# MikeWangWZHL/VidIL

Hardware: AMD Instinct MI355X
Metric: frames/sec whole-node (BLIP caption+filt + CLIP visual-token) 224^2 8f/video (higher is better)
Workload: dtype bf16

## Files before the change

### vidil_amd/csrc/common.h

```cpp
#pragma once
#include <hip/hip_runtime.h>
#include <atomic>
#include <stdint.h>
#include <stdio.h>
#include "../../include/vidil_hip.h"

typedef _Float16 f16;
typedef _Float16 f16x4 __attribute__((ext_vector_type(4)));
typedef _Float16 f16x8 __attribute__((ext_vector_type(8)));
typedef __bf16 bf16;
typedef __bf16 bf16x4 __attribute__((ext_vector_type(4)));
typedef __bf16 bf16x8 __attribute__((ext_vector_type(8)));
typedef float f32x2 __attribute__((ext_vector_type(2)));
typedef float f32x4 __attribute__((ext_vector_type(4)));
typedef float f32x16 __attribute__((ext_vector_type(16)));
typedef uint32_t u32x2 __attribute__((ext_vector_type(2)));
typedef uint32_t u32x4 __attribute__((ext_vector_type(4)));

#define VIDIL_WAVE 64

void vidil_set_error(const char* fmt, ...);
int vidil_cu_count();
int vidil_lds_opt_in(std::atomic<unsigned long long>& mask, const void* kern, int bytes, const char* who);
const char* vidil_dev_env(const char* name);

bool vidil_gemm256_eligible(const vidil_gemm_args& a, bool any_size = false);
int vidil_gemm256_launch(const vidil_gemm_args& a, hipStream_t s);
const char* vidil_gemm256_variant(const vidil_gemm_args& a);
bool vidil_gemm4w128_wanted(const vidil_gemm_args& a);
int vidil_gemm4w128_launch(const vidil_gemm_args& a, hipStream_t s);
bool vidil_gemm_c3_serves(const vidil_gemm_args& a);
int vidil_gemm4w_c3_launch(const vidil_gemm_args& a, hipStream_t s);

#define VIDIL_REQUIRE(cond, ...)                \
  do {                                          \
    if (!(cond)) {                              \
      vidil_set_error(__VA_ARGS__);             \
      return VIDIL_EINVAL;                      \
    }                                           \
  } while (0)

#define VIDIL_CHECK_LAUNCH(what)                                            \
  do {                                                                      \
    hipError_t e__ = hipGetLastError();                                     \
    if (e__ != hipSuccess) {                                                \
      vidil_set_error("%s: launch failed: %s", what, hipGetErrorString(e__)); \
      return VIDIL_ELAUNCH;                                                 \
    }                                                                       \
  } while (0)

__host__ __device__ __forceinline__ int vt_pos(int t) { return t ^ ((((t >> 2) ^ (t >> 3)) & 1) * 12); }

__host__ __device__ __forceinline__ size_t ktile_off(int t, int c) {
  return (size_t)(t >> 5) * 2048 + (size_t)(((c >> 3) * 32 + (t & 31)) * 8 + (c & 7));
}
__host__ __device__ __forceinline__ size_t vtile_off(int t, int d) {
  const int tt = t & 31, g = (tt & 15) >> 2;
  return (size_t)(t >> 5) * 2048 +
         (size_t)(((((tt >> 4) * 2 + (d >> 5)) * 2 + (g & 1)) * 32 + (d & 31)) * 8 + (g >> 1) * 4 + (tt & 3));
}

__device__ __forceinline__ float wave_sum(float v) {
#pragma unroll
  for (int o = 32; o > 0; o >>= 1) v += __shfl_xor(v, o, 64);
  return v;
}
__device__ __forceinline__ float wave_max(float v) {
#pragma unroll
  for (int o = 32; o > 0; o >>= 1) v = fmaxf(v, __shfl_xor(v, o, 64));
  return v;
}
__device__ __forceinline__ f16 to_f16(float v) {
  asm volatile("" : "+v"(v));
  return (f16)v;
}

template <typename T> struct Elt;
template <> struct Elt<f16> {
  typedef f16x4 x4;
  typedef f16x8 x8;
  static constexpr int kDtype = VIDIL_DT_F16;
  static __device__ __forceinline__ f32x16 mfma32(x8 a, x8 b, f32x16 c) { return __builtin_amdgcn_mfma_f32_32x32x16_f16(a, b, c, 0, 0, 0); }
  static __device__ __forceinline__ f16 from_f32(float v) { return to_f16(v); }
};
template <> struct Elt<bf16> {
  typedef bf16x4 x4;
  typedef bf16x8 x8;
  static constexpr int kDtype = VIDIL_DT_BF16;
  static __device__ __forceinline__ f32x16 mfma32(x8 a, x8 b, f32x16 c) { return __builtin_amdgcn_mfma_f32_32x32x16_bf16(a, b, c, 0, 0, 0); }
  static __device__ __forceinline__ bf16 from_f32(float v) {
    asm volatile("" : "+v"(v));
    return (bf16)v;
  }
};
struct fp8 { uint8_t bits; };
typedef int i32x8 __attribute__((ext_vector_type(8)));
typedef int i32x4 __attribute__((ext_vector_type(4)));
template <> struct Elt<fp8> {
  static constexpr int kDtype = VIDIL_DT_FP8;
};
__device__ __forceinline__ uint32_t pack4_fp8(float a, float b, float c, float d) {
  a = fminf(fmaxf(a, -448.f), 448.f);
  b = fminf(fmaxf(b, -448.f), 448.f);
  c = fminf(fmaxf(c, -448.f), 448.f);
  d = fminf(fmaxf(d, -448.f), 448.f);
  int w = __builtin_amdgcn_cvt_pk_fp8_f32(a, b, 0, false);
  w = __builtin_amdgcn_cvt_pk_fp8_f32(c, d, w, true);
  return (uint32_t)w;
}

template <typename T> __device__ __forceinline__ typename Elt<T>::x8 zero8() {
  typename Elt<T>::x8 z;
#pragma unroll
  for (int e = 0; e < 8; ++e) z[e] = (T)0.f;
  return z;
}
#define VIDIL_DISPATCH_DTYPE(dtype, what, ...)                                         \
  do {                                                                                 \
    if ((dtype) == VIDIL_DT_F16) { using T = f16; __VA_ARGS__; }                       \
    else if ((dtype) == VIDIL_DT_BF16) { using T = bf16; __VA_ARGS__; }                \
    else { vidil_set_error("%s: unknown dtype %d", what, (int)(dtype)); return VIDIL_EINVAL; } \
  } while (0)

__device__ __forceinline__ f32x2 pk_fma(f32x2 a, f32x2 b, f32x2 c) { return __builtin_elementwise_fma(a, b, c); }
__device__ __forceinline__ f32x2 pk_splat(float v) { return f32x2{v, v}; }
__device__ __forceinline__ f32x2 gelu_erf2(f32x2 x) {
  const f32x2 xs = x * pk_splat(0.70710678118654752440f);
  const f32x2 ax = __builtin_elementwise_abs(xs);
  const f32x2 den = pk_fma(pk_splat(0.3275911f), ax, pk_splat(1.0f));
  const f32x2 t = {__builtin_amdgcn_rcpf(den[0]), __builtin_amdgcn_rcpf(den[1])};
  f32x2 p = pk_fma(pk_splat(1.061405429f), t, pk_splat(-1.453152027f));
  p = pk_fma(p, t, pk_splat(1.421413741f));
  p = pk_fma(p, t, pk_splat(-0.284496736f));
  p = pk_fma(p, t, pk_splat(0.254829592f));
  const f32x2 arg = (ax * ax) * pk_splat(-1.4426950408889634f);
  const f32x2 e = {__builtin_amdgcn_exp2f(arg[0]), __builtin_amdgcn_exp2f(arg[1])};
  const f32x2 y = pk_fma(-(p * t), e, pk_splat(1.0f));
  const f32x2 er = {copysignf(y[0], xs[0]), copysignf(y[1], xs[1])};
  return (x * pk_splat(0.5f)) * (er + pk_splat(1.0f));
}
template <typename TO> struct GeluPoly;
template <> struct GeluPoly<f16> {
  static constexpr int DEG = 8;
  static constexpr float q[9] = {3.988192516e-01f, -6.619034771e-02f, 9.718823738e-03f, -1.079092217e-03f, 8.849158500e-05f,
                                 -5.147754456e-06f, 1.986294828e-07f, -4.515713104e-09f, 4.547582994e-11f};
};
template <> struct GeluPoly<bf16> {
  static constexpr int DEG = 6;
  static constexpr float q[7] = {3.978833846e-01f, -6.457313509e-02f, 8.772395999e-03f, -8.140167550e-04f, 4.795563103e-05f,
                                 -1.598607122e-06f, 2.278152054e-08f};
};
template <typename TO>
__device__ __forceinline__ float gelu_fast1(float x) {
  using P = GeluPoly<TO>;
  const float s = x * x;
  float p = __builtin_fmaf(P::q[P::DEG], s, P::q[P::DEG - 1]);
#pragma unroll
  for (int k = P::DEG - 2; k >= 0; --k) p = __builtin_fmaf(p, s, P::q[k]);
  const float phi = __builtin_amdgcn_fmed3f(__builtin_fmaf(x, p, 0.5f), 0.f, 1.f);
  return x * phi;
}
template <typename TO>
__device__ __forceinline__ f32x2 gelu_fast2(f32x2 x) { return f32x2{gelu_fast1<TO>(x[0]), gelu_fast1<TO>(x[1])}; }
__device__ __forceinline__ f32x2 pk_fma_half_clamp(f32x2 a, f32x2 b) {
  f32x2 d;
  asm("v_pk_fma_f32 %0, %1, %2, 0.5 op_sel_hi:[1,1,0] clamp" : "=v"(d) : "v"(a), "v"(b));
  return d;
}
template <typename TO, int NP>
__device__ __forceinline__ void gelu_fast2p_n(f32x2 (&x)[NP]) {
  using P = GeluPoly<TO>;
  f32x2 s[NP], p[NP];
#pragma unroll
  for (int i = 0; i < NP; ++i) s[i] = x[i] * x[i];
#pragma unroll
  for (int i = 0; i < NP; ++i) p[i] = pk_fma(pk_splat(P::q[P::DEG]), s[i], pk_splat(P::q[P::DEG - 1]));
#pragma unroll
  for (int k = P::DEG - 2; k >= 0; --k)
#pragma unroll
    for (int i = 0; i < NP; ++i) p[i] = pk_fma(p[i], s[i], pk_splat(P::q[k]));
#pragma unroll
// ... 12 lines not shown
```

### vidil_amd/csrc/gemm256.hip

```cpp
#include <type_traits>

#include "common.h"
#include "gemm_epilogue.h"

namespace {

constexpr int SLOT = 16384;
constexpr int BUF = 4 * SLOT;
constexpr int LDS_BYTES = 2 * BUF;
constexpr int STATS_BYTES = 2 * 4 * 128 * 8;

__device__ __forceinline__ void glds16(const void* g, char* lds) {
  __builtin_amdgcn_global_load_lds((const __attribute__((address_space(1))) void*)g,
                                   (__attribute__((address_space(3))) void*)lds, 16, 0, 0);
}

template <int EPI>
constexpr bool kPersistent = EPI != VIDIL_EPI_HEADS && EPI != VIDIL_EPI_ARENA;

#ifdef VIDIL_GEMM_PROBE
__device__ unsigned long long g_probe[2];
struct Probe {
  unsigned long long t0, r0;
  __device__ Probe() : t0(__builtin_readcyclecounter()), r0(__builtin_amdgcn_s_memrealtime()) {}
// ... 147 lines not shown
        if (ks == 0) { dma_piece(h, 0); dma_piece(h, 1); dma_piece(h, 2); }
      }
    }
  };

  auto prologue = [&]() {
    issue(baseW, gW[0], 0, 2);
    issue(baseW, gW[1], 0, 3);
    issue(baseA, gA[0], 0, 0);
    issue(baseA, gA[1], 0, 1);
  };
  prologue();

  for (;;) {
#pragma unroll
  for (int it = 0; it < 4; ++it)
#pragma unroll
    for (int j = 0; j < 2; ++j)
#pragma unroll
      for (int r = 0; r < 16; ++r) acc[it][j][r] = 0.f;
  if constexpr (ROWSTAT) {
    const int nparts = (FOLD ? K : N) >> 6;
    const f32x2* stats_in = (const f32x2*)p.ln_stats;
    const int part0 = wc + 4 * hi;
#pragma unroll
    for (int it = 0; it < 4; ++it) {
      int row = m0 + grp * 128 + it * 32 + l31;
      row = row < M ? row : M - 1;
      st_raw[it][0] = part0 < nparts ? stats_in[(size_t)row * nparts + part0] : f32x2{0.f, 0.f};
      st_raw[it][1] = part0 + 8 < nparts ? stats_in[(size_t)row * nparts + part0 + 8] : f32x2{0.f, 0.f};
    }
  }

  int h = 0;
  if (grp == 1) {
    sync(h);
    dma_piece(h, 0); dma_piece(h, 1); dma_piece(h, 2);
    ++h;
  }
  for (int u = 0; u < nk; ++u) {
    const char* buf = smem + (u & 1) * BUF;
    sync(h);
    half_period(std::integral_constant<int, 0>{}, buf, h);
    ++h;
    sync(h);
    half_period(std::integral_constant<int, 1>{}, buf, h);
    ++h;
  }
  if (grp == 0) sync(h);
  asm volatile("s_waitcnt vmcnt(0) lgkmcnt(0)" ::: "memory");
  __builtin_amdgcn_s_barrier();

  if constexpr (ROWSTAT) {
    f32x2* stats = (f32x2*)(smem + LDS_BYTES);
#pragma unroll
    for (int it = 0; it < 4; ++it) {
      const float s0 = st_raw[it][0][0] + st_raw[it][1][0], ss0 = st_raw[it][0][1] + st_raw[it][1][1];
      const float s = s0 + __shfl_xor(s0, 32, 64);
      const float ss = ss0 + __shfl_xor(ss0, 32, 64);
      if (hi == 0) stats[(grp * 4 + wc) * 128 + it * 32 + l31] = f32x2{s, ss};
    }
    asm volatile("s_waitcnt lgkmcnt(0)" ::: "memory");
    __builtin_amdgcn_s_barrier();
    const float inv_k = 1.0f / (float)(FOLD ? K : N);
#pragma unroll
    for (int it = 0; it < 4; ++it) {
      float s = 0.f, ss = 0.f;
#pragma unroll
      for (int w = 0; w < 4; ++w) {
        const f32x2 v = stats[(grp * 4 + w) * 128 + it * 32 + l31];
        s += v[0];
        ss += v[1];
      }
      const float mean = s * inv_k;
      float var = ss * inv_k - mean * mean;
      var = var > 0.f ? var : 0.f;
      const float rstd = 1.0f / sqrtf(var + p.ln_eps);
      st_s[it] = rstd;
      st_ss[it] = mean * rstd;
    }
  }

  const int m_w = m0 + grp * 128;
  const int n_w = n0 + wc * 64;
  const bool more = kPersistent<EPI> && ESZ == 2 && !RLN && remaining > tile_step;
  if (more) {
    logical += tile_step;
    remaining -= tile_step;
    setup_tile(logical);
    prologue();
  }
  do {
    char* const ep = smem + BUF + wave * 8192;
#include "gemm_epilogue.inc"
  } while (0);
  if (!more) break;
  asm volatile("s_waitcnt vmcnt(0) lgkmcnt(0)" ::: "memory");
  }
}

template <typename T, int EPI, int ACT, bool FOLD = false, typename TO = T, bool STATS = false, bool RLN = false>
int launch256(const vidil_gemm_args& a, hipStream_t s) {
  static std::atomic<unsigned long long> attr_set{0};
  auto kern = gemm256_kernel<T, TO, EPI, ACT, FOLD, STATS, RLN>;
  constexpr int lds = LDS_BYTES + ((FOLD || RLN) ? STATS_BYTES : 0);
  if (const int rc_ = vidil_lds_opt_in(attr_set, (const void*)kern, lds, "gemm256")) return rc_;
  const int num_cu = vidil_cu_count() & ~7;
  const int ntiles = ((a.M + 255) / 256) * ((a.N + 255) / 256);
  const int tiles = !(kPersistent<EPI> && sizeof(T) == 2 && !RLN) ? ntiles : ntiles >= num_cu ? num_cu : (ntiles >= 8 ? ((ntiles + 7) & ~7) : ntiles);
  hipLaunchKernelGGL(kern, dim3(tiles), dim3(512), lds, s, a);
  VIDIL_CHECK_LAUNCH("gemm256");
  return VIDIL_OK;
}

}

#ifdef VIDIL_GEMM_PROBE
extern "C" int vidil_debug_gemm_probe(unsigned long long* out2) {
  return hipMemcpyFromSymbol(out2, HIP_SYMBOL(g_probe), 16) == hipSuccess ? 0 : -1;
}
#endif

bool vidil_gemm256_eligible(const vidil_gemm_args& a, bool any_size) {
  const long tiles = (long)((a.M + 255) / 256) * ((a.N + 255) / 256);
  if (tiles < 5L * vidil_cu_count() / 8 && !any_size) return false;
  if (a.K < 128) return false;
  if (a.dtype == VIDIL_DT_FP8 && (a.K % 128 != 0 || (a.lda != 0 && a.lda % 16 != 0))) return false;
  const long lda = a.lda > 0 ? a.lda : a.K;
  if (256L * lda >= (1L << 31) || (long)a.N * a.K >= (1L << 31)) return false;
  auto al16 = [](const void* p) { return ((uintptr_t)p & 15) == 0; };
  if (a.bias && !al16(a.bias)) return false;
  if (a.ln_fold && !(a.ln_colsum && al16(a.ln_colsum) && a.N % 4 == 0 && a.ln_stats && ((uintptr_t)a.ln_stats & 7) == 0)) return false;
  if (a.ln_stats_out && !(a.N % 64 == 0 && ((uintptr_t)a.ln_stats_out & 7) == 0)) return false;
  if (a.w_scale && !al16(a.w_scale)) return false;
  switch (a.epi) {
    case VIDIL_EPI_F8:
      return a.dtype == VIDIL_DT_FP8 && a.N % 16 == 0 && a.ldo % 16 == 0 && al16(a.out);
    case VIDIL_EPI_F16:
      return a.N % 8 == 0 && a.ldo % 8 == 0 && al16(a.out);
    case VIDIL_EPI_F32:
      if (a.out16 && !(a.ldo16 % 4 == 0 && ((uintptr_t)a.out16 & 7) == 0)) return false;
      return a.N % 4 == 0 && a.ldo % 4 == 0 && al16(a.out) && (!a.resid || al16(a.resid));
    case VIDIL_EPI_PATCH:
      return a.N % 4 == 0 && a.ldo % 4 == 0 && al16(a.out) && al16(a.pos);
    case VIDIL_EPI_HEADS:
      return (!a.q || al16(a.q)) && (!a.k || al16(a.k)) && ((a.NP != 0 && !a.kv_tiled) || !a.vt || al16(a.vt));
    case VIDIL_EPI_ARENA:
      return (!a.q || al16(a.q)) && (!a.k || al16(a.k)) && (!a.vt || al16(a.vt));
    default:
      return false;
  }
}

template <typename T>
static int launch256_dispatch(const vidil_gemm_args& a, hipStream_t s) {
  if (a.ln_fold) {
    if (a.epi == VIDIL_EPI_HEADS) return launch256<T, VIDIL_EPI_HEADS, VIDIL_ACT_NONE, true>(a, s);
    if (a.epi == VIDIL_EPI_ARENA) return launch256<T, VIDIL_EPI_ARENA, VIDIL_ACT_NONE, true>(a, s);
    if (a.act == VIDIL_ACT_NONE) return launch256<T, VIDIL_EPI_F16, VIDIL_ACT_NONE, true>(a, s);
    if (a.act == VIDIL_ACT_GELU_ERF) return launch256<T, VIDIL_EPI_F16, VIDIL_ACT_GELU_ERF, true>(a, s);
    return launch256<T, VIDIL_EPI_F16, VIDIL_ACT_QUICK_GELU, true>(a, s);
  }
  switch (a.epi) {
    case VIDIL_EPI_F16:
      if (a.act == VIDIL_ACT_NONE) return launch256<T, VIDIL_EPI_F16, VIDIL_ACT_NONE>(a, s);
      if (a.act == VIDIL_ACT_GELU_ERF) return launch256<T, VIDIL_EPI_F16, VIDIL_ACT_GELU_ERF>(a, s);
      return launch256<T, VIDIL_EPI_F16, VIDIL_ACT_QUICK_GELU>(a, s);
    case VIDIL_EPI_F32:
      if (a.rln_gamma) return launch256<T, VIDIL_EPI_F32, VIDIL_ACT_NONE, false, T, true, true>(a, s);
      if (a.ln_stats_out) return launch256<T, VIDIL_EPI_F32, VIDIL_ACT_NONE, false, T, true>(a, s);
      if (a.act == VIDIL_ACT_NONE) return launch256<T, VIDIL_EPI_F32, VIDIL_ACT_NONE>(a, s);
      if (a.act == VIDIL_ACT_GELU_ERF) return launch256<T, VIDIL_EPI_F32, VIDIL_ACT_GELU_ERF>(a, s);
      return launch256<T, VIDIL_EPI_F32, VIDIL_ACT_QUICK_GELU>(a, s);
    case VIDIL_EPI_HEADS:
      return launch256<T, VIDIL_EPI_HEADS, VIDIL_ACT_NONE>(a, s);
    case VIDIL_EPI_ARENA:
      return launch256<T, VIDIL_EPI_ARENA, VIDIL_ACT_NONE>(a, s);
    default:
      return launch256<T, VIDIL_EPI_PATCH, VIDIL_ACT_NONE>(a, s);
  }
}

template <typename TO>
static int launch256_fp8(const vidil_gemm_args& a, hipStream_t s) {
  switch (a.epi) {
    case VIDIL_EPI_F32: return launch256<fp8, VIDIL_EPI_F32, VIDIL_ACT_NONE, false, TO>(a, s);
    case VIDIL_EPI_PATCH: return launch256<fp8, VIDIL_EPI_PATCH, VIDIL_ACT_NONE, false, TO>(a, s);
    case VIDIL_EPI_HEADS: return launch256<fp8, VIDIL_EPI_HEADS, VIDIL_ACT_NONE, false, TO>(a, s);
    case VIDIL_EPI_F8:
      if (a.act == VIDIL_ACT_GELU_ERF) return launch256<fp8, VIDIL_EPI_F8, VIDIL_ACT_GELU_ERF, false, TO>(a, s);
      if (a.act == VIDIL_ACT_QUICK_GELU) return launch256<fp8, VIDIL_EPI_F8, VIDIL_ACT_QUICK_GELU, false, TO>(a, s);
      return launch256<fp8, VIDIL_EPI_F8, VIDIL_ACT_NONE, false, TO>(a, s);
    default:
      vidil_set_error("gemm/fp8: epilogue %d is not built for fp8 operands", a.epi);
      return VIDIL_EUNSUP;
  }
}

int vidil_gemm4w_launch(const vidil_gemm_args& a, hipStream_t s, int tm);

static bool prefer_4w(const vidil_gemm_args& a) {
  if (a.epi == VIDIL_EPI_HEADS && a.T < 8) return false;
  if (const char* e = vidil_dev_env("VIDIL_GEMM4W")) return atoi(e) != 0;
  const long tiles = (long)((a.M + 255) / 256) * ((a.N + 255) / 256);
  static const long min_tiles = 3L * vidil_cu_count() / 2;
  if (a.dtype == VIDIL_DT_FP8) {
    return tiles >= min_tiles &&
           (a.epi == VIDIL_EPI_F8 || a.epi == VIDIL_EPI_HEADS || (a.epi == VIDIL_EPI_F32 && a.act == VIDIL_ACT_NONE));
  }
  if (tiles < min_tiles) return false;
  if (a.ln_fold) return true;
  switch (a.epi) {
    case VIDIL_EPI_F16:
    case VIDIL_EPI_HEADS:
    case VIDIL_EPI_ARENA:
      return true;
    case VIDIL_EPI_F32: {
      return a.ln_stats_out != nullptr || a.K >= 1536;
    }
    default:
      return false;
  }
}

const char* vidil_gemm256_variant(const vidil_gemm_args& a) { return prefer_4w(a) ? "gemm4w_kernel" : "gemm256_kernel"; }

bool vidil_gemm4w128_wanted(const vidil_gemm_args& a) {
  const char* e = vidil_dev_env("VIDIL_GEMM4W128");
  const int mode = e ? atoi(e) : -1;
  if (mode == 0 || a.dtype == VIDIL_DT_FP8 || a.ln_fold || a.ln_stats_out || a.rln_gamma || a.out16) return false;
  if (a.epi == VIDIL_EPI_HEADS && a.T < 8) return false;
  if (!(a.epi == VIDIL_EPI_F16 || a.epi == VIDIL_EPI_HEADS || a.epi == VIDIL_EPI_ARENA || (a.epi == VIDIL_EPI_F32 && a.act == VIDIL_ACT_NONE)))
    return false;
  if (!vidil_gemm256_eligible(a, true)) return false;
  if (mode == 1) return true;
  const long t256 = (long)((a.M + 255) / 256) * ((a.N + 255) / 256);
  const long t128 = (long)((a.M + 127) / 128) * ((a.N + 255) / 256);
  return t256 < 5L * vidil_cu_count() / 8 && t128 >= 25L * vidil_cu_count() / 32 && a.K >= 512;
}
int vidil_gemm4w128_launch(const vidil_gemm_args& a, hipStream_t s) { return vidil_gemm4w_launch(a, s, 2); }

int vidil_gemm256_launch(const vidil_gemm_args& a, hipStream_t s) {
  if (prefer_4w(a)) {
    const int rc = vidil_gemm4w_launch(a, s, 4);
    if (rc != -1000) return rc;
  }
  if (a.dtype == VIDIL_DT_FP8) return a.dtype16 == VIDIL_DT_BF16 ? launch256_fp8<bf16>(a, s) : launch256_fp8<f16>(a, s);
  if (a.dtype == VIDIL_DT_BF16) return launch256_dispatch<bf16>(a, s);
  return launch256_dispatch<f16>(a, s);
}
```

### vidil_amd/csrc/gemm_epilogue.inc

```
  if (n_w >= N) break;

#ifdef VIDIL_EPI_NIT
  constexpr int NIT = VIDIL_EPI_NIT;
#else
  constexpr int NIT = 4;
#endif
#ifdef VIDIL_EPI_LAZY
  f32x4 q_b[2][4], q_c[2][4];
  const bool has_bias = p.bias != nullptr;
#pragma unroll
  for (int j = 0; j < 2; ++j)
#pragma unroll
    for (int rq = 0; rq < 4; ++rq) {
      q_b[j][rq] = f32x4{0.f, 0.f, 0.f, 0.f};
      q_c[j][rq] = f32x4{0.f, 0.f, 0.f, 0.f};
    }
#ifdef VIDIL_EPI_BIAS_LDS
  constexpr bool VEC_LDS = EPI == VIDIL_EPI_F16 || EPI == VIDIL_EPI_HEADS || EPI == VIDIL_EPI_ARENA || EPI == VIDIL_EPI_F8;
#else
  constexpr bool VEC_LDS = false;
#endif
  if constexpr (VEC_LDS) {
#ifdef VIDIL_EPI_BIAS_LDS
    if (has_bias) {
#pragma unroll
      for (int j = 0; j < 2; ++j)
#pragma unroll
        for (int rq = 0; rq < 4; ++rq) q_b[j][rq] = *(const f32x4*)(epb + (j * 32 + rq * 8 + hi * 4) * 4);
    }
    if constexpr (FOLD || ESZ == 1) {
#pragma unroll
      for (int j = 0; j < 2; ++j)
#pragma unroll
        for (int rq = 0; rq < 4; ++rq) q_c[j][rq] = *(const f32x4*)(epb + 512 + (j * 32 + rq * 8 + hi * 4) * 4);
    }
#endif
  } else {
    if (has_bias) {
#pragma unroll
      for (int j = 0; j < 2; ++j)
#pragma unroll
        for (int rq = 0; rq < 4; ++rq) {
          const int col = n_w + j * 32 + rq * 8 + hi * 4;
          q_b[j][rq] = *(const f32x4*)(p.bias + (col + 4 <= N ? col : N - 4));
        }
    }
    if constexpr (FOLD || ESZ == 1) {
      const float* const cvec = FOLD ? p.ln_colsum : p.w_scale;
#pragma unroll
      for (int j = 0; j < 2; ++j)
#pragma unroll
        for (int rq = 0; rq < 4; ++rq) {
          const int col = n_w + j * 32 + rq * 8 + hi * 4;
          q_c[j][rq] = *(const f32x4*)(cvec + (col + 4 <= N ? col : N - 4));
        }
    }
  }
  auto quadrow = [&](int it, int j, f32x4 (&q4)[4]) {
    f32x2 w[8];
#pragma unroll
    for (int pi = 0; pi < 8; ++pi) {
      const int rq = pi >> 1, e = (pi & 1) * 2;
      w[pi] = f32x2{acc[it][j][rq * 4 + e], acc[it][j][rq * 4 + e + 1]};
      const f32x2 b2 = {q_b[j][rq][e], q_b[j][rq][e + 1]};
      if constexpr (FOLD) {
        const f32x2 c2 = {q_c[j][rq][e], q_c[j][rq][e + 1]};
        w[pi] = pk_fma(w[pi], pk_splat(st_s[it]), pk_fma(pk_splat(-st_ss[it]), c2, b2));
      } else if constexpr (ESZ == 1) {
        const f32x2 c2 = {q_c[j][rq][e], q_c[j][rq][e + 1]};
        w[pi] = pk_fma(w[pi], c2, b2);
      } else {
        w[pi] = w[pi] + b2;
      }
    }
    if constexpr (ACT == VIDIL_ACT_GELU_ERF && EPI != VIDIL_EPI_F32) {
      gelu_fast2p_n<TO, 8>(w);
    } else if constexpr (ACT != VIDIL_ACT_NONE) {
#pragma unroll
      for (int pi = 0; pi < 8; ++pi) w[pi] = ACT == VIDIL_ACT_GELU_ERF ? gelu_erf2(w[pi]) : quick_gelu2(w[pi]);
    }
#pragma unroll
    for (int rq = 0; rq < 4; ++rq) q4[rq] = f32x4{w[rq * 2][0], w[rq * 2][1], w[rq * 2 + 1][0], w[rq * 2 + 1][1]};
  };
#else
  if constexpr (FOLD) {
#pragma unroll
    for (int j = 0; j < 2; ++j)
#pragma unroll
      for (int rq = 0; rq < 4; ++rq) {
        const int col = n_w + j * 32 + rq * 8 + hi * 4;
        if (col + 4 <= N) {
          const f32x4 c4 = *(const f32x4*)(p.ln_colsum + col);
          f32x4 b4 = {0.f, 0.f, 0.f, 0.f};
          if (p.bias != nullptr) b4 = *(const f32x4*)(p.bias + col);
#pragma unroll
          for (int it = 0; it < 4; ++it)
#pragma unroll
            for (int e = 0; e < 4; ++e)
              acc[it][j][rq * 4 + e] = __builtin_fmaf(acc[it][j][rq * 4 + e], st_s[it], __builtin_fmaf(-st_ss[it], c4[e], b4[e]));
        }
      }
  } else if constexpr (ESZ == 1) {
#pragma unroll
    for (int j = 0; j < 2; ++j)
#pragma unroll
      for (int rq = 0; rq < 4; ++rq) {
        const int col = n_w + j * 32 + rq * 8 + hi * 4;
        if (col + 4 <= N) {
          const f32x4 w4 = *(const f32x4*)(p.w_scale + col);
          f32x4 b4 = {0.f, 0.f, 0.f, 0.f};
          if (p.bias != nullptr) b4 = *(const f32x4*)(p.bias + col);
#pragma unroll
          for (int it = 0; it < 4; ++it)
#pragma unroll
            for (int e = 0; e < 4; ++e) acc[it][j][rq * 4 + e] = __builtin_fmaf(acc[it][j][rq * 4 + e], w4[e], b4[e]);
        }
      }
  } else
  if (p.bias != nullptr) {
#pragma unroll
    for (int j = 0; j < 2; ++j)
#pragma unroll
      for (int rq = 0; rq < 4; ++rq) {
        const int col = n_w + j * 32 + rq * 8 + hi * 4;
        if (col + 4 <= N) {
          const f32x4 b4 = *(const f32x4*)(p.bias + col);
#pragma unroll
          for (int it = 0; it < 4; ++it)
#pragma unroll
            for (int e = 0; e < 4; ++e) acc[it][j][rq * 4 + e] += b4[e];
        }
      }
  }
  if constexpr (ACT != VIDIL_ACT_NONE) {
#pragma unroll
    for (int it = 0; it < 4; ++it)
#pragma unroll
      for (int j = 0; j < 2; ++j)
#pragma unroll
        for (int r = 0; r < 16; r += 2) {
          f32x2 v = {acc[it][j][r], acc[it][j][r + 1]};
          v = ACT == VIDIL_ACT_GELU_ERF ? (EPI == VIDIL_EPI_F32 ? gelu_erf2(v) : gelu_fast2<TO>(v)) : quick_gelu2(v);
          acc[it][j][r] = v[0];
          acc[it][j][r + 1] = v[1];
        }
  }
  auto quadrow = [&](int it, int j, f32x4 (&q4)[4]) {
#pragma unroll
    for (int rq = 0; rq < 4; ++rq) q4[rq] = f32x4{acc[it][j][rq * 4 + 0], acc[it][j][rq * 4 + 1], acc[it][j][rq * 4 + 2], acc[it][j][rq * 4 + 3]};
  };
#endif

  int part = 0, head = 0;
  if constexpr (EPI == VIDIL_EPI_HEADS || EPI == VIDIL_EPI_ARENA) {
    const int hd = p.H * 64;
    part = p.part0 + n_w / hd;
    head = (n_w % hd) >> 6;
  }

  if constexpr (EPI == VIDIL_EPI_HEADS) {
    if (part == 2 && p.kv_tiled) {
      constexpr int ROWB = 136;
      const size_t img_stride = (size_t)p.H * p.Tk_cap * 64;
      f16* const vbase = (f16*)p.vt + (size_t)head * p.Tk_cap * 64;
#pragma unroll
      for (int it = 0; it < NIT; ++it) {
        const int mb = m_w + it * 32;
        const int rows = M - mb < 32 ? M - mb : 32;
        if (rows <= 0) break;
#pragma unroll
        for (int j = 0; j < 2; ++j) {
          f32x4 q4[4];
          quadrow(it, j, q4);
#pragma unroll
          for (int rq = 0; rq < 4; ++rq) {
            const f32x4 q = q4[rq];
            const f16x4 v = {Elt<TO>::from_f32(q[0]), Elt<TO>::from_f32(q[1]), Elt<TO>::from_f32(q[2]), Elt<TO>::from_f32(q[3])};
            *(f16x4*)(ep + l31 * ROWB + (j * 32 + rq * 8 + hi * 4) * 2) = v;
          }
        }
        int b = mb / p.T, t = mb - b * p.T;
        for (int r = 0; r < rows;) {
          const int tt = p.t_off + t;
          f16* dst = vbase + (size_t)b * img_stride + vtile_off(tt, lane);
          const char* src = ep + r * ROWB + lane * 2;
          if ((tt & 3) == 0 && r + 4 <= rows && t + 4 <= p.T) {
            const f16x4 v = {*(const f16*)src, *(const f16*)(src + ROWB), *(const f16*)(src + 2 * ROWB),
                             *(const f16*)(src + 3 * ROWB)};
            *(f16x4*)dst = v;
            r += 4;
            t += 4;
          } else {
            *dst = *(const f16*)src;
            r += 1;
            t += 1;
          }
          if (t >= p.T) { t -= p.T; ++b; }
        }
      }
      break;
    }
    if (part == 2 && p.NP != 0) {
#pragma unroll
      for (int it = 0; it < NIT; ++it) {
        const int m = m_w + it * 32 + l31;
        if (m < M) {
          const int b = m / p.T, t = m - b * p.T;
          f16* dst = (f16*)p.vt + (((size_t)b * p.H + head) * 64) * (size_t)p.NP + vt_pos(p.t_off + t);
#pragma unroll
          for (int j = 0; j < 2; ++j) {
            f32x4 q4[4];
            quadrow(it, j, q4);
#pragma unroll
            for (int rq = 0; rq < 4; ++rq) {
              const f32x4 q = q4[rq];
#pragma unroll
              for (int e = 0; e < 4; ++e) dst[(size_t)(j * 32 + rq * 8 + hi * 4 + e) * p.NP] = Elt<TO>::from_f32(q[e]);
            }
          }
        }
      }
      break;
    }
  }

  if constexpr (EPI == VIDIL_EPI_F8) {
#pragma unroll
    for (int pass = 0; pass < 2; ++pass) {
#pragma unroll
      for (int i = 0; i < 2; ++i) {
        const int it = pass * 2 + i;
        const int row = i * 32 + l31;
#pragma unroll
        for (int j = 0; j < 2; ++j) {
          f32x4 q4[4];
          quadrow(it, j, q4);
#pragma unroll
          for (int rq = 0; rq < 4; ++rq) {
            const int cb = j * 32 + rq * 8 + hi * 4;
            const f32x4 q = q4[rq];
            *(uint32_t*)(ep + row * 64 + ((((cb >> 4) ^ ((row >> 2) & 3)) << 4) | (cb & 15))) = pack4_fp8(q[0], q[1], q[2], q[3]);
          }
        }
      }
      const int ch = lane & 3;
#ifdef VIDIL_EPI_LAZY
      const uint32_t pitch8 = (uint32_t)p.ldo;
      const int rows_w8 = M - m_w < 32 * NIT ? M - m_w : 32 * NIT;
      const __amdgpu_buffer_rsrc_t r_o8 = uniform_rsrc((char*)p.out + (size_t)m_w * p.ldo + n_w, (rows_w8 > 0 ? (uint32_t)rows_w8 : 0u) * pitch8);
      uint32_t vo8 = n_w + ch * 16 + 16 <= N ? (uint32_t)(pass * 64 + (lane >> 2)) * pitch8 + (uint32_t)ch * 16u : 0x80000000u;
#pragma unroll
      for (int iter = 0; iter < 4; ++iter) {
        const int row = iter * 16 + (lane >> 2);
        const u32x4 v = *(const u32x4*)(ep + row * 64 + ((ch ^ ((row >> 2) & 3)) << 4));
        __builtin_amdgcn_raw_buffer_store_b128(v, r_o8, vo8, 0, 0);
        vo8 += 16u * pitch8;
      }
#else
#pragma unroll
      for (int iter = 0; iter < 4; ++iter) {
        const int row = iter * 16 + (lane >> 2);
        const i32x4 v = *(const i32x4*)(ep + row * 64 + ((ch ^ ((row >> 2) & 3)) << 4));
        const int m = m_w + pass * 64 + row;
        const int col = n_w + ch * 16;
        if (m < M && col + 16 <= N) *(i32x4*)((char*)p.out + (size_t)m * p.ldo + col) = v;
      }
#endif
    }
  } else if constexpr (EPI == VIDIL_EPI_F16 || EPI == VIDIL_EPI_HEADS || EPI == VIDIL_EPI_ARENA) {
    const float scale = ((EPI == VIDIL_EPI_HEADS || EPI == VIDIL_EPI_ARENA) && part == 0) ? p.q_scale : 1.0f;
#ifdef VIDIL_EPI_LAZY
    {
      const int ch = lane & 7;
      auto compute_write = [&](int it, char* buf) {
#pragma unroll
        for (int j = 0; j < 2; ++j) {
          f32x4 q4[4];
          quadrow(it, j, q4);
#pragma unroll
          for (int rq = 0; rq < 4; ++rq) {
            const f32x4 q = q4[rq];
            const f32x2 q01 = f32x2{q[0], q[1]} * pk_splat(scale), q23 = f32x2{q[2], q[3]} * pk_splat(scale);
            const f16x4 v = {Elt<TO>::from_f32(q01[0]), Elt<TO>::from_f32(q01[1]), Elt<TO>::from_f32(q23[0]), Elt<TO>::from_f32(q23[1])};
            *(f16x4*)(buf + l31 * 128 + (((j * 4 + rq) ^ (l31 & 7)) << 4) + hi * 8) = v;
          }
        }
      };
      auto read_rows = [&](const char* buf, f16x8 (&v4)[4]) {
#pragma unroll
        for (int i = 0; i < 4; ++i) {
          const int row = i * 8 + (lane >> 3);
          v4[i] = *(const f16x8*)(buf + row * 128 + ((ch ^ (row & 7)) << 4));
        }
      };
      f16* hb = nullptr;
      int cap = 0, toff = 0;
      bool tiled = false;
      size_t img = 0;
      if constexpr (EPI == VIDIL_EPI_HEADS) {
        if (part == 0) { hb = (f16*)p.q; cap = p.Tq_cap; toff = 0; tiled = false; }
        else { hb = (f16*)(part == 1 ? p.k : p.vt); cap = p.Tk_cap; toff = p.t_off; tiled = p.kv_tiled != 0; }
        hb += (size_t)head * cap * 64;
        img = (size_t)p.H * cap * 64;
      }
      if constexpr (EPI == VIDIL_EPI_ARENA) {
        hb = (f16*)(part == 0 ? p.q : part == 1 ? p.k : p.vt) + head * 64;
      }
      const bool colok = n_w + ch * 8 + 8 <= N;
      __amdgpu_buffer_rsrc_t r_o16;
      uint32_t vo_o16 = 0, step_o16 = 0;
      if constexpr (EPI == VIDIL_EPI_F16) {
        const uint32_t pitch = (uint32_t)p.ldo * (uint32_t)sizeof(f16);
        const int rows_w = M - m_w < 32 * NIT ? M - m_w : 32 * NIT;
        r_o16 = uniform_rsrc((char*)p.out + ((size_t)m_w * p.ldo + n_w) * sizeof(f16), (rows_w > 0 ? (uint32_t)rows_w : 0u) * pitch);
        vo_o16 = colok ? (uint32_t)(lane >> 3) * pitch + (uint32_t)ch * 16u : 0x80000000u;
        step_o16 = 8u * pitch;
      }
      __amdgpu_buffer_rsrc_t r_hd;
      int hs_b = 0, hs_t = 0, hs_b0 = 0;
      uint32_t img_b = 0;
      if constexpr (EPI == VIDIL_EPI_HEADS) {
        const int b0 = m_w / p.T;
        hs_b0 = b0;
        r_hd = uniform_rsrc((char*)(hb + (size_t)b0 * img), 0x80000000u);
        const int m0l = m_w + (lane >> 3);
        const int bb = m0l / p.T;
        hs_t = m0l - bb * p.T;
        hs_b = bb - b0;
        img_b = (uint32_t)(img * sizeof(f16));
      }
      auto store_rows = [&](int it, f16x8 (&v4)[4]) {
        const int m_first = m_w + it * 32 + (lane >> 3);
        if constexpr (EPI == VIDIL_EPI_F16) {
#pragma unroll
          for (int i = 0; i < 4; ++i) {
            __builtin_amdgcn_raw_buffer_store_b128(__builtin_bit_cast(u32x4, v4[i]), r_o16, vo_o16, 0, 0);
            vo_o16 += step_o16;
          }
        } else if constexpr (EPI == VIDIL_EPI_HEADS) {
          auto rows4 = [&](auto tiled_tag) {
            constexpr bool TILED = decltype(tiled_tag)::value;
#pragma unroll
            for (int i = 0; i < 4; ++i) {
              const int m = m_first + i * 8;
              const uint32_t e = TILED ? (uint32_t)ktile_off(toff + hs_t, ch * 8) : (uint32_t)(toff + hs_t) * 64u + (uint32_t)ch * 8u;
              uint32_t off = (uint32_t)hs_b * img_b + e * (uint32_t)sizeof(f16);
              off = (m < M && colok) ? off : 0x80000000u;
              __builtin_amdgcn_raw_buffer_store_b128(__builtin_bit_cast(u32x4, v4[i]), r_hd, off, 0, 0);
              hs_t += 8;
              const bool wrap = hs_t >= p.T;
              hs_t = wrap ? hs_t - p.T : hs_t;
              hs_b = wrap ? hs_b + 1 : hs_b;
            }
          };
          if (tiled) {
            rows4(std::true_type{});
          } else {
            rows4(std::false_type{});
          }
        } else {
          int b = m_first / p.T, t = m_first - b * p.T;
          const size_t hd = (size_t)p.H * 64;
#pragma unroll
          for (int i = 0; i < 4; ++i) {
            const int m = m_first + i * 8;
            if (m < M && colok) {
              f16* d = hb + (part == 0 ? (size_t)m : (size_t)(p.t_off + t) * p.arena_rows + (size_t)b * p.slot_stride) * hd + ch * 8;
              *(f16x8*)d = v4[i];
            }
            t += 8;
            while (t >= p.T) { t -= p.T; ++b; }
          }
        }
      };
      f16x8 vr[4];
      compute_write(0, ep);
#pragma unroll
      for (int it = 1; it < NIT; ++it) {
        read_rows(ep, vr);
        __builtin_amdgcn_sched_barrier(0);
        compute_write(it, ep);
        __builtin_amdgcn_sched_barrier(0);
        store_rows(it - 1, vr);
        __builtin_amdgcn_sched_barrier(0);
      }
      read_rows(ep, vr);
      store_rows(NIT - 1, vr);
    }
#else
#pragma unroll
    for (int pass = 0; pass < 2; ++pass) {
#pragma unroll
      for (int i = 0; i < 2; ++i) {
        const int it = pass * 2 + i;
        const int row = i * 32 + l31;
#pragma unroll
        for (int j = 0; j < 2; ++j) {
          f32x4 q4[4];
          quadrow(it, j, q4);
#pragma unroll
          for (int rq = 0; rq < 4; ++rq) {
            const f32x4 q = q4[rq];
            const f16x4 v = {Elt<TO>::from_f32(q[0] * scale), Elt<TO>::from_f32(q[1] * scale), Elt<TO>::from_f32(q[2] * scale),
                             Elt<TO>::from_f32(q[3] * scale)};
            *(f16x4*)(ep + row * 128 + (((j * 4 + rq) ^ (row & 7)) << 4) + hi * 8) = v;
          }
        }
      }
      const int ch = lane & 7;
#pragma unroll 4
      for (int iter = 0; iter < 8; ++iter) {
        const int row = iter * 8 + (lane >> 3);
        const f16x8 v = *(const f16x8*)(ep + row * 128 + ((ch ^ (row & 7)) << 4));
        const int m = m_w + pass * 64 + row;
        const int col = n_w + ch * 8;
        if (m < M && col + 8 <= N) {
          if constexpr (EPI == VIDIL_EPI_F16) {
            *(f16x8*)((f16*)p.out + (size_t)m * p.ldo + col) = v;
          } else if constexpr (EPI == VIDIL_EPI_ARENA) {
            const int b = m / p.T, t = m - b * p.T;
            const size_t hd = (size_t)p.H * 64;
            f16* base = (f16*)(part == 0 ? p.q : part == 1 ? p.k : p.vt) + head * 64 + ch * 8;
            *(f16x8*)(base + (part == 0 ? (size_t)m : (size_t)(p.t_off + t) * p.arena_rows + (size_t)b * p.slot_stride) * hd) = v;
          } else {
            const int b = m / p.T, t = m - b * p.T;
            const size_t bh = (size_t)b * p.H + head;
            if (part == 0) {
              *(f16x8*)((f16*)p.q + (bh * p.Tq_cap + t) * 64 + ch * 8) = v;
            } else {
              f16* kv = (f16*)(part == 1 ? p.k : p.vt);
              if (p.kv_tiled) {
                *(f16x8*)(kv + bh * p.Tk_cap * 64 + ktile_off(p.t_off + t, ch * 8)) = v;
              } else {
                *(f16x8*)(kv + (bh * p.Tk_cap + p.t_off + t) * 64 + ch * 8) = v;
              }
            }
          }
        }
      }
    }
#endif
  } else {
    f32x4 rln_g = {1.f, 1.f, 1.f, 1.f}, rln_b = {0.f, 0.f, 0.f, 0.f};
    if constexpr (RLN) {
      const int col = n_w + (lane & 15) * 4;
      if (col + 4 <= N) {
        rln_g = *(const f32x4*)(p.rln_gamma + col);
        rln_b = *(const f32x4*)(p.rln_beta + col);
      }
    }
    if constexpr (EPI == VIDIL_EPI_F32) {
#ifndef VIDIL_EPI_F32_AHEAD
#define VIDIL_EPI_F32_AHEAD 1
#endif
      constexpr int AH = VIDIL_EPI_F32_AHEAD;
      const int ch = lane & 15;
      const uint32_t pitch = (uint32_t)p.ldo * 4u;
      const int rows_w = M - m_w < 32 * NIT ? M - m_w : 32 * NIT;
      const uint32_t nrows = rows_w > 0 ? (uint32_t)rows_w : 0u;
      const size_t e0 = (size_t)m_w * p.ldo + n_w;
      const bool has_res = p.resid != nullptr, has16 = p.out16 != nullptr;
      const bool s3 = !STATS && !RLN && p.out16_split3 != 0;
      const bool s3_third = p.out16_split3 != 2;
      const uint32_t pl16 = (uint32_t)(p.ldo16 / 3) * 2u;
      const __amdgpu_buffer_rsrc_t r_out = uniform_rsrc((char*)p.out + e0 * 4, p.out != nullptr ? nrows * pitch : 0u);
      const __amdgpu_buffer_rsrc_t r_res = uniform_rsrc((const char*)(has_res ? p.resid : (const float*)p.out) + e0 * 4, has_res ? nrows * pitch : 0u);
      const uint32_t pitch16 = (uint32_t)p.ldo16 * 2u;
      const __amdgpu_buffer_rsrc_t r_16 = uniform_rsrc((char*)p.out16 + (has16 ? ((size_t)m_w * p.ldo16 + n_w) * 2 : 0), has16 ? nrows * pitch16 : 0u);
      const bool colok = n_w + ch * 4 + 4 <= N;
      const uint32_t vo0 = colok ? (uint32_t)(lane >> 4) * pitch + (uint32_t)ch * 16u : 0x80000000u;
      const uint32_t vo16_0 = colok ? (uint32_t)(lane >> 4) * pitch16 + (uint32_t)ch * 8u : 0x80000000u;
      f32x4 addb[AH + 1][8];
      uint32_t vo_ld = vo0, vo_st = vo0, vo16 = vo16_0;
      const uint32_t step = 4u * pitch, step16 = 4u * pitch16;
      auto load_rows = [&](f32x4 (&a8)[8]) {
#pragma unroll
        for (int iter = 0; iter < 8; ++iter) {
          a8[iter] = __builtin_bit_cast(f32x4, __builtin_amdgcn_raw_buffer_load_b128(r_res, vo_ld, 0, 0));
          vo_ld += step;
        }
      };
#pragma unroll
      for (int a = 0; a < AH; ++a)
        if (a < NIT) load_rows(addb[a]);
#pragma unroll
      for (int pass = 0; pass < NIT; ++pass) {
        if (pass + AH < NIT) load_rows(addb[(pass + AH) % (AH + 1)]);
        {
          const int it = pass;
          const int lr = l31;
#pragma unroll
          for (int j = 0; j < 2; ++j) {
            f32x4 q4[4];
            quadrow(it, j, q4);
#pragma unroll
            for (int rq = 0; rq < 4; ++rq) *(f32x4*)(ep + lr * 256 + (((j * 8 + rq * 2 + hi) ^ (lr & 7)) << 4)) = q4[rq];
          }
        }
        f32x4 vrow[8];
#pragma unroll
        for (int iter = 0; iter < 8; ++iter) {
          const int lr = iter * 4 + (lane >> 4);
          vrow[iter] = *(const f32x4*)(ep + lr * 256 + ((ch ^ (lr & 7)) << 4));
        }
        float rs8[8], mrs8[8];
        if constexpr (RLN) {
#pragma unroll
          for (int iter = 0; iter < 8; ++iter) {
            const int lr = iter * 4 + (lane >> 4);
            rs8[iter] = __shfl(st_s[pass], lr, 64);
            mrs8[iter] = __shfl(st_ss[pass], lr, 64);
          }
        }
        float part[16];
#pragma unroll
        for (int iter = 0; iter < 8; ++iter) {
          f32x4 v = vrow[iter];
          {
            f32x4 ad = addb[pass % (AH + 1)][iter];
            if constexpr (RLN) {
              const float rs = rs8[iter], mrs = mrs8[iter];
#pragma unroll
              for (int e = 0; e < 4; ++e) ad[e] = __builtin_fmaf(__builtin_fmaf(ad[e], rs, -mrs), rln_g[e], rln_b[e]);
            }
// ... 211 lines not shown
```

Measured before the change: 5136.

## Use buffer stores with running offsets in HEADS/ARENA epilogues for small T

Rewrites the GEMM epilogue row stores for the HEADS and ARENA paths to use buffer-resource stores with precomputed running byte offsets, stepping rows with a batch/time stride so sequence lengths below 8 work. This lets the 4-wave GEMM paths serve HEADS with T<8 (previously excluded), gated by a new check that the arena offset span fits in 31 bits. It also adds an optional lazy V-tile scatter path behind a compile flag. The goal is less per-row index division and branching in the store loop, and more shapes on the faster kernel. The cost is more complex offset arithmetic that could be wrong on edge cases.

```diff
diff --git a/vidil_amd/csrc/common.h b/vidil_amd/csrc/common.h
--- a/vidil_amd/csrc/common.h
+++ b/vidil_amd/csrc/common.h
@@ -27,6 +27,7 @@
 bool vidil_gemm256_eligible(const vidil_gemm_args& a, bool any_size = false);
 int vidil_gemm256_launch(const vidil_gemm_args& a, hipStream_t s);
 const char* vidil_gemm256_variant(const vidil_gemm_args& a);
+bool vidil_gemm4w_arena_fits(const vidil_gemm_args& a);
 bool vidil_gemm4w128_wanted(const vidil_gemm_args& a);
 int vidil_gemm4w128_launch(const vidil_gemm_args& a, hipStream_t s);
 bool vidil_gemm_c3_serves(const vidil_gemm_args& a);
diff --git a/vidil_amd/csrc/gemm256.hip b/vidil_amd/csrc/gemm256.hip
--- a/vidil_amd/csrc/gemm256.hip
+++ b/vidil_amd/csrc/gemm256.hip
@@ -323,6 +323,13 @@
   }
 }
 
+bool vidil_gemm4w_arena_fits(const vidil_gemm_args& a) {
+  if (a.epi != VIDIL_EPI_ARENA || a.T <= 0 || a.H <= 0) return true;
+  if (a.part0 == 0 && a.N <= a.H * 64) return true;
+  const long long span = ((long long)(a.T - 1) * a.arena_rows + (long long)(256 / a.T + 2) * a.slot_stride) * a.H * 128LL;
+  return span < (1LL << 31);
+}
+
 template <typename T>
 static int launch256_dispatch(const vidil_gemm_args& a, hipStream_t s) {
   if (a.ln_fold) {
@@ -371,7 +378,7 @@
 int vidil_gemm4w_launch(const vidil_gemm_args& a, hipStream_t s, int tm);
 
 static bool prefer_4w(const vidil_gemm_args& a) {
-  if (a.epi == VIDIL_EPI_HEADS && a.T < 8) return false;
+  if (!vidil_gemm4w_arena_fits(a)) return false;
   if (const char* e = vidil_dev_env("VIDIL_GEMM4W")) return atoi(e) != 0;
   const long tiles = (long)((a.M + 255) / 256) * ((a.N + 255) / 256);
   static const long min_tiles = 3L * vidil_cu_count() / 2;
@@ -400,7 +407,7 @@
   const char* e = vidil_dev_env("VIDIL_GEMM4W128");
   const int mode = e ? atoi(e) : -1;
   if (mode == 0 || a.dtype == VIDIL_DT_FP8 || a.ln_fold || a.ln_stats_out || a.rln_gamma || a.out16) return false;
-  if (a.epi == VIDIL_EPI_HEADS && a.T < 8) return false;
+  if (!vidil_gemm4w_arena_fits(a)) return false;
   if (!(a.epi == VIDIL_EPI_F16 || a.epi == VIDIL_EPI_HEADS || a.epi == VIDIL_EPI_ARENA || (a.epi == VIDIL_EPI_F32 && a.act == VIDIL_ACT_NONE)))
     return false;
   if (!vidil_gemm256_eligible(a, true)) return false;
diff --git a/vidil_amd/csrc/gemm_epilogue.inc b/vidil_amd/csrc/gemm_epilogue.inc
--- a/vidil_amd/csrc/gemm_epilogue.inc
+++ b/vidil_amd/csrc/gemm_epilogue.inc
@@ -163,6 +163,12 @@
       constexpr int ROWB = 136;
       const size_t img_stride = (size_t)p.H * p.Tk_cap * 64;
       f16* const vbase = (f16*)p.vt + (size_t)head * p.Tk_cap * 64;
+#ifdef VIDIL_EPI_LAZY
+      const int vb0 = m_w / p.T;
+      int vs_t = m_w - vb0 * p.T, vs_b = 0;
+      const uint32_t img_b = (uint32_t)(img_stride * sizeof(f16));
+      const __amdgpu_buffer_rsrc_t r_v = uniform_rsrc((char*)(vbase + (size_t)vb0 * img_stride), 0x80000000u);
+#endif
 #pragma unroll
       for (int it = 0; it < NIT; ++it) {
         const int mb = m_w + it * 32;
@@ -179,6 +185,44 @@
             *(f16x4*)(ep + l31 * ROWB + (j * 32 + rq * 8 + hi * 4) * 2) = v;
           }
         }
+#ifdef VIDIL_EPI_LAZY
+        {
+          const int q = lane >> 3, dl = lane & 7;
+          int lo = 0;
+          do {
+            const int hi_r = lo + (p.T - vs_t) < rows ? lo + (p.T - vs_t) : rows;
+            const int key0 = p.t_off + vs_t - lo;
+            const uint32_t imgoff = (uint32_t)vs_b * img_b;
+            const int r0 = 4 * q - (key0 & 3);
+            const bool full = r0 >= lo && r0 + 4 <= hi_r;
+            const char* src8 = ep + (r0 < 0 ? 0 : r0) * ROWB + dl * 2;
+            f16x4 v8[8];
+#pragma unroll
+            for (int i = 0; i < 8; ++i)
+              v8[i] = f16x4{*(const f16*)(src8 + i * 16), *(const f16*)(src8 + ROWB + i * 16), *(const f16*)(src8 + 2 * ROWB + i * 16),
+                            *(const f16*)(src8 + 3 * ROWB + i * 16)};
+            const int c = lane >> 3;
+            const int r = c < 3 ? lo + c : hi_r - 6 + c;
+            const int gs = r - ((key0 + r) & 3);
+            const bool single = c < 6 && r >= lo && r < hi_r && (c < 3 || r >= lo + 3) && !(gs >= lo && gs + 4 <= hi_r);
+            const char* src2 = ep + (r < 0 ? 0 : r > 31 ? 31 : r) * ROWB + dl * 2;
+            f16 v2[8];
+#pragma unroll
+            for (int i = 0; i < 8; ++i) v2[i] = *(const f16*)(src2 + i * 16);
+            const uint32_t off8 = full ? imgoff + (uint32_t)vtile_off(key0 + r0, dl) * 2u : 0x80000000u;
+            const uint32_t off2 = single ? imgoff + (uint32_t)vtile_off(key0 + r, dl) * 2u : 0x80000000u;
+#pragma unroll
+            for (int i = 0; i < 8; ++i)
+              __builtin_amdgcn_raw_buffer_store_b64(__builtin_bit_cast(u32x2, v8[i]), r_v, off8 + (uint32_t)((i >> 2) * 1024 + (i & 3) * 128), 0, 0);
+#pragma unroll
+            for (int i = 0; i < 8; ++i)
+              __builtin_amdgcn_raw_buffer_store_b16(__builtin_bit_cast(short, v2[i]), r_v, off2 + (uint32_t)((i >> 2) * 1024 + (i & 3) * 128), 0, 0);
+            vs_t += hi_r - lo;
+            lo = hi_r;
+            if (vs_t >= p.T) { vs_t = 0; ++vs_b; }
+          } while (lo < rows);
+        }
+#else
         int b = mb / p.T, t = mb - b * p.T;
         for (int r = 0; r < rows;) {
           const int tt = p.t_off + t;
@@ -197,6 +241,7 @@
           }
           if (t >= p.T) { t -= p.T; ++b; }
         }
+#endif
       }
       break;
     }
@@ -317,59 +362,91 @@
         step_o16 = 8u * pitch;
       }
       __amdgpu_buffer_rsrc_t r_hd;
-      int hs_b = 0, hs_t = 0, hs_b0 = 0;
+      int hs_b = 0, hs_t = 0;
       uint32_t img_b = 0;
-      if constexpr (EPI == VIDIL_EPI_HEADS) {
-        const int b0 = m_w / p.T;
-        hs_b0 = b0;
-        r_hd = uniform_rsrc((char*)(hb + (size_t)b0 * img), 0x80000000u);
+      uint32_t lin_off = 0, lin_step = 0, lin_wrap = 0;
+      int seq_t = 1;
+      if constexpr (EPI == VIDIL_EPI_HEADS || EPI == VIDIL_EPI_ARENA) {
+        seq_t = p.T;
+        asm volatile("" : "+s"(seq_t));
+      }
+      const int st_a = seq_t > 8 ? 0 : seq_t >= 5 ? 1 : seq_t >= 3 ? 2 : seq_t == 2 ? 4 : 8;
+      const int st_r = 8 - st_a * seq_t;
+      if constexpr (EPI == VIDIL_EPI_HEADS || EPI == VIDIL_EPI_ARENA) {
+        const int b0 = m_w / seq_t;
         const int m0l = m_w + (lane >> 3);
-        const int bb = m0l / p.T;
-        hs_t = m0l - bb * p.T;
+        const int bb = m0l / seq_t;
+        hs_t = m0l - bb * seq_t;
         hs_b = bb - b0;
-        img_b = (uint32_t)(img * sizeof(f16));
+        uint32_t pitch_b = 0, pitch_t = 0;
+        if constexpr (EPI == VIDIL_EPI_HEADS) {
+          r_hd = uniform_rsrc((char*)(hb + (size_t)b0 * img), 0x80000000u);
+          img_b = (uint32_t)(img * sizeof(f16));
+          pitch_b = img_b;
+          pitch_t = 128u;
+          lin_off = (uint32_t)toff * 128u;
+        } else if (part == 0) {
+          const uint32_t pitch = (uint32_t)p.H * 128u;
+          const int rows_w = M - m_w < 32 * NIT ? M - m_w : 32 * NIT;
+          r_hd = uniform_rsrc((char*)(hb + (size_t)m_w * p.H * 64), (rows_w > 0 ? (uint32_t)rows_w : 0u) * pitch);
+          lin_off = colok ? (uint32_t)(lane >> 3) * pitch + (uint32_t)ch * 16u : 0x80000000u;
+          lin_step = 8u * pitch;
+        } else {
+          const size_t hd = (size_t)p.H * 64;
+          r_hd = uniform_rsrc((char*)(hb + ((size_t)p.t_off * p.arena_rows + (size_t)b0 * p.slot_stride) * hd), 0x80000000u);
+          pitch_b = (uint32_t)p.slot_stride * (uint32_t)p.H * 128u;
+          pitch_t = (uint32_t)p.arena_rows * (uint32_t)p.H * 128u;
+        }
+        if (EPI == VIDIL_EPI_HEADS || part != 0) {
+          lin_off += (uint32_t)hs_b * pitch_b + (uint32_t)hs_t * pitch_t + (uint32_t)ch * 16u;
+          lin_step = (uint32_t)st_a * pitch_b + (uint32_t)st_r * pitch_t;
+          lin_wrap = pitch_b - (uint32_t)seq_t * pitch_t;
+        }
       }
       auto store_rows = [&](int it, f16x8 (&v4)[4]) {
         const int m_first = m_w + it * 32 + (lane >> 3);
+        auto rows4_running = [&](const __amdgpu_buffer_rsrc_t& r, uint32_t& vo, uint32_t step) {
+#pragma unroll
+          for (int i = 0; i < 4; ++i) {
+            __builtin_amdgcn_raw_buffer_store_b128(__builtin_bit_cast(u32x4, v4[i]), r, vo, 0, 0);
+            vo += step;
+          }
+        };
+        auto rows4_linear = [&]() {
+#pragma unroll
+          for (int i = 0; i < 4; ++i) {
+            const int m = m_first + i * 8;
+            __builtin_amdgcn_raw_buffer_store_b128(__builtin_bit_cast(u32x4, v4[i]), r_hd, (m < M && colok) ? lin_off : 0x80000000u, 0, 0);
+            hs_t += st_r;
+            const bool wrap = hs_t >= seq_t;
+            hs_t = wrap ? hs_t - seq_t : hs_t;
+            lin_off += lin_step + (wrap ? lin_wrap : 0u);
+          }
+        };
         if constexpr (EPI == VIDIL_EPI_F16) {
-#pragma unroll
-          for (int i = 0; i < 4; ++i) {
-            __builtin_amdgcn_raw_buffer_store_b128(__builtin_bit_cast(u32x4, v4[i]), r_o16, vo_o16, 0, 0);
-            vo_o16 += step_o16;
-          }
+          rows4_running(r_o16, vo_o16, step_o16);
         } else if constexpr (EPI == VIDIL_EPI_HEADS) {
-          auto rows4 = [&](auto tiled_tag) {
-            constexpr bool TILED = decltype(tiled_tag)::value;
+          if (tiled) {
 #pragma unroll
             for (int i = 0; i < 4; ++i) {
               const int m = m_first + i * 8;
-              const uint32_t e = TILED ? (uint32_t)ktile_off(toff + hs_t, ch * 8) : (uint32_t)(toff + hs_t) * 64u + (uint32_t)ch * 8u;
-              uint32_t off = (uint32_t)hs_b * img_b + e * (uint32_t)sizeof(f16);
+              uint32_t off = (uint32_t)hs_b * img_b + (uint32_t)ktile_off(toff + hs_t, ch * 8) * (uint32_t)sizeof(f16);
               off = (m < M && colok) ? off : 0x80000000u;
               __builtin_amdgcn_raw_buffer_store_b128(__builtin_bit_cast(u32x4, v4[i]), r_hd, off, 0, 0);
-              hs_t += 8;
-              const bool wrap = hs_t >= p.T;
-              hs_t = wrap ? hs_t - p.T : hs_t;
+              hs_t += st_r;
+              hs_b += st_a;
+              const bool wrap = hs_t >= seq_t;
+              hs_t = wrap ? hs_t - seq_t : hs_t;
               hs_b = wrap ? hs_b + 1 : hs_b;
             }
-          };
-          if (tiled) {
-            rows4(std::true_type{});
           } else {
-            rows4(std::false_type{});
+            rows4_linear();
           }
         } else {
-          int b = m_first / p.T, t = m_first - b * p.T;
-          const size_t hd = (size_t)p.H * 64;
-#pragma unroll
-          for (int i = 0; i < 4; ++i) {
-            const int m = m_first + i * 8;
-            if (m < M && colok) {
-              f16* d = hb + (part == 0 ? (size_t)m : (size_t)(p.t_off + t) * p.arena_rows + (size_t)b * p.slot_stride) * hd + ch * 8;
-              *(f16x8*)d = v4[i];
-            }
-            t += 8;
-            while (t >= p.T) { t -= p.T; ++b; }
+          if (part == 0) {
+            rows4_running(r_hd, lin_off, lin_step);
+          } else {
+            rows4_linear();
           }
         }
       };
```

Result: no change. 5160, median of 6 (+0.5%).
